# Ronnypetson/epivo

Hardware: NVIDIA B200
Metric: KITTI-shape frame-pairs/sec (match+E-RANSAC+pose+LM) (higher is better)
Workload: dtype u32-popc+f64

## Files before the change

epivo_b200/csrc/seq.cu:

```cuda
#include <stdlib.h>
#include <string.h>

#include <algorithm>
#include <vector>

#include "common.cuh"
#include "stages.cuh"

namespace {
constexpr int SEQ_CHUNK = 8192;
constexpr int SEQ_CHUNK_OVERLAP = 1024;
constexpr int SEQ_STAGES = 7;
constexpr int SEQ_MAX_CHUNKS = 256;
}

struct epivo_seq {
    epivo_ctx* ctx = nullptr;
    int max_frames = 0, kp = 0, stride = 0, chunk = SEQ_CHUNK;
    float* d_kps = nullptr;
    uint32_t* d_desc = nullptr;
    uint32_t* d_planes = nullptr;
    int32_t* d_counts = nullptr;
    bool counts_set = false;
    int32_t *d_fq = nullptr, *d_ft = nullptr;
    bool pairs_set = false;
    int max_pairs = 0, n_list = 0;
    int frames_hi = 0;
    int list_max = 0;
    std::vector<int32_t> h_fq, h_ft;
    int32_t *d_mq = nullptr, *d_mt = nullptr, *d_md = nullptr, *d_nmatch = nullptr;
    uint8_t *d_emask = nullptr, *d_pmask = nullptr;
    double *d_E = nullptr, *d_R = nullptr, *d_t = nullptr, *d_T = nullptr, *d_T0 = nullptr;
    int32_t *d_ninl = nullptr, *d_iters = nullptr, *d_nmodels = nullptr, *d_status = nullptr, *d_ngood = nullptr;
    int32_t *d_lmactive = nullptr, *d_lmiters = nullptr;
    epivo_lm_res* d_lmres = nullptr;
    epivo_pair_result* d_results = nullptr;
    uint32_t *d_rowkey = nullptr, *d_rowkey2 = nullptr, *d_colkey = nullptr;
    double *d_xn = nullptr, *d_xin = nullptr, *d_lmp = nullptr, *d_lmq = nullptr, *d_w = nullptr;
    float* d_err = nullptr;
    int32_t* d_reps = nullptr;
    char* d_esswork = nullptr;
    size_t esswork_bytes = 0;
    epivo_pair_result* h_results = nullptr;
    cudaEvent_t ev[SEQ_MAX_CHUNKS][SEQ_STAGES] = {};
    cudaEvent_t evk[SEQ_MAX_CHUNKS][2] = {};
    cudaEvent_t evp[SEQ_MAX_CHUNKS] = {};
    cudaEvent_t ev_begin = nullptr, ev_end = nullptr;
    cudaStream_t stream2 = nullptr;
    cudaStream_t stream3 = nullptr;
    cudaStream_t stream4 = nullptr;
    cudaEvent_t ev_piece[SEQ_MAX_CHUNKS] = {};
    int geo_mode = 0;
    cudaEvent_t ev_matched[SEQ_MAX_CHUNKS] = {};
    cudaEvent_t ev_geo_done = nullptr;
    int overlap = 0;
    int match_pad = 0;
    int last_mgroups = 0, last_ggroups = 0;
    int last_n_pairs = 0, last_first = 0;
    float* d_trk = nullptr;
    bool last_frames = false;
    std::vector<void*> allocs;
};

namespace {

template <typename T>
int seq_alloc(epivo_seq* s, T** p, size_t count) {
    epivo_ctx* ctx = s->ctx;
    void* q = nullptr;
    EPV_CUDA(ctx, cudaMalloc(&q, std::max<size_t>(count, 1) * sizeof(T)));
    s->allocs.push_back(q);
    *p = reinterpret_cast<T*>(q);
    return EPIVO_OK;
}

__global__ void lm_prep_kernel(int n_pairs, int stride, epivo_pipeline_params prm, const double* __restrict__ R,
                               const double* __restrict__ t, const int32_t* __restrict__ status,
                               const int32_t* __restrict__ n_inl, const int32_t* __restrict__ n_good,
                               const double* __restrict__ xin, double* __restrict__ T0, double* __restrict__ T,
                               double* __restrict__ lmp, double* __restrict__ lmq, double* __restrict__ w,
                               int32_t* __restrict__ active) {
    const int pair = blockIdx.x;
    if (pair >= n_pairs) return;
    const int tid = threadIdx.x;
    const int N = prm.lm_points;
    __shared__ double sT[16];
    if (tid == 0) {
        double Rm[9], tv[3];
        for (int i = 0; i < 9; ++i) Rm[i] = R[(int64_t)pair * 9 + i];
        for (int i = 0; i < 3; ++i) tv[i] = t[(int64_t)pair * 3 + i];
        const bool ok = status[pair] == 0;
        if (!ok || (Rm[0] + Rm[4] + Rm[8]) < prm.min_trace) {
            for (int i = 0; i < 9; ++i) Rm[i] = (i % 4 == 0) ? 1.0 : 0.0;
            for (int i = 0; i < 3; ++i) tv[i] = prm.fallback_t[i];
        }
        if (sqrt(tv[0] * tv[0] + tv[1] * tv[1] + tv[2] * tv[2]) < prm.min_t_norm)
            for (int i = 0; i < 3; ++i) tv[i] = prm.fallback_t[i];
        for (int i = 0; i < 3; ++i) {
            for (int j = 0; j < 3; ++j) sT[i * 4 + j] = Rm[i * 3 + j];
            sT[i * 4 + 3] = tv[i];
        }
        sT[12] = sT[13] = sT[14] = 0.0;
        sT[15] = 1.0;
        active[pair] = (ok && n_inl[pair] >= N && n_good[pair] >= N) ? 1 : 0;
        w[pair] = 1.0;
    }
    __syncthreads();
    if (tid < 16) {
        T0[(int64_t)pair * 16 + tid] = sT[tid];
        T[(int64_t)pair * 16 + tid] = sT[tid];
    }
    const double* x = xin + (int64_t)pair * 4 * stride;
    for (int i = tid; i < N; i += blockDim.x) {
        const bool have = i < n_inl[pair];
        double* p = lmp + ((int64_t)pair * N + i) * 3;
        double* q = lmq + ((int64_t)pair * N + i) * 3;
        p[0] = have ? x[i] : 1.0;
        p[1] = have ? x[stride + i] : 1.0;
        p[2] = 1.0;
        q[0] = have ? x[2 * stride + i] : 1.0;
        q[1] = have ? x[3 * stride + i] : 1.0;
        q[2] = 1.0;
    }
}

__device__ __forceinline__ double knorm(float u, double a, double b) { return __fma_rn((double)u, a, b); }

__global__ void __launch_bounds__(256) points_in_kernel(const float* __restrict__ p0, const float* __restrict__ p1,
                                                        const int32_t* __restrict__ counts, int max_pts, int stride,
                                                        double ax, double bx, double ay, double by,
                                                        double* __restrict__ xn, int32_t* __restrict__ nmatch,
                                                        int32_t* __restrict__ mq, int32_t* __restrict__ mt) {
    const int pair = blockIdx.y, i = blockIdx.x * 256 + threadIdx.x;
    const int n = min(max(counts[pair], 0), max_pts);
    if (i == 0) nmatch[pair] = n;
    if (i >= n) return;
    const float2 a = reinterpret_cast<const float2*>(p0)[(size_t)pair * max_pts + i];
    const float2 b = reinterpret_cast<const float2*>(p1)[(size_t)pair * max_pts + i];
    double* x = xn + (size_t)pair * 4 * stride;
    x[i] = knorm(a.x, ax, bx);
    x[stride + i] = knorm(a.y, ay, by);
    x[2 * stride + i] = knorm(b.x, ax, bx);
    x[3 * stride + i] = knorm(b.y, ay, by);
    mq[(size_t)pair * stride + i] = i;
    mt[(size_t)pair * stride + i] = i;
}

__global__ void __launch_bounds__(256) track_compact_kernel(const int32_t* __restrict__ meta, int n, const float* __restrict__ kps,
                                                            const int32_t* __restrict__ found, int kp,
                                                            const float* __restrict__ next, const uint8_t* __restrict__ status,
                                                            int stride, double ax, double bx, double ay, double by,
                                                            float* __restrict__ trk, double* __restrict__ xn,
                                                            int32_t* __restrict__ nmatch, int32_t* __restrict__ mq,
                                                            int32_t* __restrict__ mt, int32_t* __restrict__ md) {
    __shared__ int s_warp[8];
    __shared__ int s_carry;
    const int j = blockIdx.x, tid = threadIdx.x, lane = tid & 31, warp = tid >> 5;
    const int fq = meta[j], pair = meta[2 * n + j];
    const int cnt = min(found[fq], kp);
    const float2* c = reinterpret_cast<const float2*>(kps) + (size_t)fq * kp;
    const float2* nx = reinterpret_cast<const float2*>(next) + (size_t)j * kp;
    const uint8_t* st = status + (size_t)j * kp;
    float2* t0 = reinterpret_cast<float2*>(trk) + (size_t)pair * 2 * stride;
    float2* t1 = t0 + stride;
    double* x = xn + (size_t)pair * 4 * stride;
    const size_t mo = (size_t)pair * stride;
    if (tid == 0) s_carry = 0;
    __syncthreads();
    for (int base = 0; base < cnt; base += 256) {
        const int i = base + tid;
        const bool keep = i < cnt && st[i] == 1;
        const unsigned bal = __ballot_sync(0xFFFFFFFFu, keep);
        if (lane == 0) s_warp[warp] = __popc(bal);
        __syncthreads();
// ... 52 lines not shown
    r.lm_iters = ran ? lmiters[pair] : 0;
    r.lm_ran = ran ? 1 : 0;
    r.lm_reverted = revert ? 1 : 0;
    out[pair] = r;
}

}

extern "C" {

void epivo_pipeline_params_default(epivo_pipeline_params* p) {
    if (!p) return;
    memset(p, 0, sizeof(*p));
    p->norm = EPIVO_NORM_HAMMING2;
    p->match_mode = EPIVO_MATCH_CROSSCHECK;
    p->ratio = 0.8f;
    const double K[9] = {(double)718.8560f, 0.0, (double)607.1928f, 0.0, (double)718.8560f, (double)185.2157f,
                         0.0, 0.0, 1.0};
    memcpy(p->K, K, sizeof(K));
    p->method = EPIVO_RANSAC;
    p->prob = 0.99;
    p->threshold = 1.0;
    p->max_iters = 1000;
    p->dist_thresh = 50.0;
    p->min_trace = 3.0 * 0.9;
    p->fallback_t[0] = 0.1;
    p->fallback_t[1] = 0.1;
    p->fallback_t[2] = -0.9;
    p->min_t_norm = 1e-5;
    p->lm_points = 48;
    p->lm_lambda0 = 1e-2;
    p->lm_epsilon = 1e-8;
    p->lm_max_iters = 30;
    p->huber_delta = 1e-5;
    p->lm_revert = 1e-9;
}

int epivo_seq_create(epivo_ctx* ctx, epivo_seq** out, int max_frames, int kp_per_frame) {
    return epivo_seq_create_pairs(ctx, out, max_frames, kp_per_frame, max_frames - 1);
}

int epivo_seq_create_pairs(epivo_ctx* ctx, epivo_seq** out, int max_frames, int kp_per_frame, int max_pairs) {
    if (!ctx || !out) return EPIVO_ERR_INVALID;
    *out = nullptr;
    if (max_frames < 2 || kp_per_frame < 1) EPV_FAIL(ctx, EPIVO_ERR_INVALID, "need >= 2 frames and >= 1 keypoint");
    if (max_pairs < max_frames - 1) EPV_FAIL(ctx, EPIVO_ERR_INVALID, "max_pairs %d < max_frames - 1", max_pairs);
    if (kp_per_frame > (int)EPV_IDX_MASK) EPV_FAIL(ctx, EPIVO_ERR_UNSUPPORTED, "too many keypoints per frame");
    EPV_CUDA(ctx, cudaSetDevice(ctx->device));
    epivo_seq* s = new epivo_seq();
    s->ctx = ctx;
    s->max_frames = max_frames;
    s->kp = kp_per_frame;
    s->stride = (kp_per_frame + 31) / 32 * 32;
    s->max_pairs = max_pairs;
    s->n_list = max_frames - 1;
    const size_t F = max_frames, P = max_pairs, st = s->stride, kp = kp_per_frame;
    s->chunk = (int)std::min<size_t>(SEQ_CHUNK, P);
    const size_t C = P;
    int rc = 0;
#define A(ptr, count) if (!rc) rc = seq_alloc(s, &s->ptr, (count))
    A(d_kps, F * kp * 2);
    A(d_desc, F * kp * 8);
    A(d_planes, F * kp * 8);
    A(d_counts, F);
    A(d_fq, P); A(d_ft, P);
    A(d_mq, P * st); A(d_mt, P * st); A(d_md, P * st); A(d_nmatch, P);
    A(d_emask, P * st); A(d_pmask, P * st);
    A(d_E, P * 9); A(d_R, P * 9); A(d_t, P * 3); A(d_T, P * 16); A(d_T0, P * 16);
    A(d_ninl, P); A(d_iters, P); A(d_nmodels, P); A(d_status, P); A(d_ngood, P);
    A(d_lmactive, P); A(d_lmiters, P); A(d_lmres, P); A(d_results, P);
    A(d_rowkey, C * st); A(d_rowkey2, C * st); A(d_colkey, C * st);
    A(d_xn, C * 4 * st); A(d_xin, C * 4 * st);
    A(d_lmp, C * 64 * 3); A(d_lmq, C * 64 * 3); A(d_w, C);
    A(d_err, epv_essential_errbuf_floats((int)C, (int)st));
    A(d_reps, 2);
    s->esswork_bytes = epv_essential_work_bytes((int)std::min<size_t>(P, SEQ_CHUNK));
    A(d_esswork, s->esswork_bytes);
#undef A
    if (!rc && cudaMallocHost(&s->h_results, P * sizeof(epivo_pair_result)) != cudaSuccess) rc = EPIVO_ERR_CUDA;
    bool ev_ok = true;
    for (int c = 0; c < SEQ_MAX_CHUNKS && ev_ok; ++c)
    {
        for (int k = 0; k < SEQ_STAGES; ++k) ev_ok &= cudaEventCreate(&s->ev[c][k]) == cudaSuccess;
        for (int k = 0; k < 2; ++k) ev_ok &= cudaEventCreate(&s->evk[c][k]) == cudaSuccess;
        ev_ok &= cudaEventCreate(&s->evp[c]) == cudaSuccess;
    }
    for (int c = 0; c < SEQ_MAX_CHUNKS && ev_ok; ++c)
        ev_ok &= cudaEventCreateWithFlags(&s->ev_matched[c], cudaEventDisableTiming) == cudaSuccess;
    ev_ok = ev_ok && cudaEventCreate(&s->ev_begin) == cudaSuccess && cudaEventCreate(&s->ev_end) == cudaSuccess;
    ev_ok = ev_ok && cudaEventCreateWithFlags(&s->ev_geo_done, cudaEventDisableTiming) == cudaSuccess;
    {
        int lo = 0, hi = 0;
        cudaDeviceGetStreamPriorityRange(&lo, &hi);
        ev_ok = ev_ok && cudaStreamCreateWithPriority(&s->stream2, cudaStreamNonBlocking, hi) == cudaSuccess;
        ev_ok = ev_ok && cudaStreamCreateWithFlags(&s->stream3, cudaStreamNonBlocking) == cudaSuccess;
        ev_ok = ev_ok && cudaStreamCreateWithPriority(&s->stream4, cudaStreamNonBlocking, hi) == cudaSuccess;
        for (int c = 0; c < SEQ_MAX_CHUNKS && ev_ok; ++c)
            ev_ok &= cudaEventCreateWithFlags(&s->ev_piece[c], cudaEventDisableTiming) == cudaSuccess;
    }
    if (rc || !ev_ok) {
        epivo_seq_destroy(s);
        if (!rc) EPV_FAIL(ctx, EPIVO_ERR_CUDA, "event creation failed");
        return rc;
    }
    const int32_t reps[2] = {0, 0};
    EPV_CUDA(ctx, cudaMemcpyAsync(s->d_reps, reps, 8, cudaMemcpyHostToDevice, ctx->stream));
    {
        std::vector<int32_t> full((size_t)max_frames, kp_per_frame);
        EPV_CUDA(ctx, cudaMemcpyAsync(s->d_counts, full.data(), full.size() * 4, cudaMemcpyHostToDevice, ctx->stream));
        EPV_CUDA(ctx, cudaStreamSynchronize(ctx->stream));
    }
    rc = epivo_seq_set_pairs(s, 0, nullptr, nullptr);
    if (rc) { epivo_seq_destroy(s); return rc; }
    s->pairs_set = false;
    EPV_CUDA(ctx, cudaStreamSynchronize(ctx->stream));
    *out = s;
    return EPIVO_OK;
}

void epivo_seq_destroy(epivo_seq* s) {
    if (!s) return;
    cudaSetDevice(s->ctx->device);
    cudaStreamSynchronize(s->ctx->stream);
    for (void* p : s->allocs) cudaFree(p);
    if (s->h_results) cudaFreeHost(s->h_results);
    for (int c = 0; c < SEQ_MAX_CHUNKS; ++c)
        for (int k = 0; k < SEQ_STAGES; ++k)
            if (s->ev[c][k]) cudaEventDestroy(s->ev[c][k]);
    for (int c = 0; c < SEQ_MAX_CHUNKS; ++c)
        for (int k = 0; k < 2; ++k)
            if (s->evk[c][k]) cudaEventDestroy(s->evk[c][k]);
    for (int c = 0; c < SEQ_MAX_CHUNKS; ++c)
        if (s->evp[c]) cudaEventDestroy(s->evp[c]);
    for (int c = 0; c < SEQ_MAX_CHUNKS; ++c)
        if (s->ev_matched[c]) cudaEventDestroy(s->ev_matched[c]);
    if (s->ev_geo_done) cudaEventDestroy(s->ev_geo_done);
    if (s->stream2) { cudaStreamSynchronize(s->stream2); cudaStreamDestroy(s->stream2); }
    if (s->stream3) { cudaStreamSynchronize(s->stream3); cudaStreamDestroy(s->stream3); }
    if (s->stream4) { cudaStreamSynchronize(s->stream4); cudaStreamDestroy(s->stream4); }
    for (int c = 0; c < SEQ_MAX_CHUNKS; ++c)
        if (s->ev_piece[c]) cudaEventDestroy(s->ev_piece[c]);
    if (s->ev_begin) cudaEventDestroy(s->ev_begin);
    if (s->ev_end) cudaEventDestroy(s->ev_end);
    delete s;
}

int epivo_seq_upload(epivo_seq* s, int first_frame, int n_frames, const float* kps, const uint8_t* descs) {
    if (!s) return EPIVO_ERR_INVALID;
    epivo_ctx* ctx = s->ctx;
    if (first_frame < 0 || n_frames < 0 || first_frame + n_frames > s->max_frames || !kps || !descs)
        EPV_FAIL(ctx, EPIVO_ERR_INVALID, "frame range [%d,+%d) outside [0,%d)", first_frame, n_frames, s->max_frames);
    EPV_CUDA(ctx, cudaSetDevice(ctx->device));
    const size_t kp = s->kp;
    EPV_CUDA(ctx, cudaMemcpyAsync(s->d_kps + (size_t)first_frame * kp * 2, kps, (size_t)n_frames * kp * 8,
                                  cudaMemcpyHostToDevice, ctx->stream));
    EPV_CUDA(ctx, cudaMemcpyAsync(s->d_desc + (size_t)first_frame * kp * 8, descs, (size_t)n_frames * kp * 32,
                                  cudaMemcpyHostToDevice, ctx->stream));
    s->frames_hi = std::max(s->frames_hi, first_frame + n_frames);
    return EPIVO_OK;
}

int epivo_seq_set_pairs(epivo_seq* s, int n_pairs, const int32_t* fq, const int32_t* ft) {
    if (!s) return EPIVO_ERR_INVALID;
    epivo_ctx* ctx = s->ctx;
    std::vector<int32_t> h;
    if (n_pairs <= 0 || !fq || !ft) {
        n_pairs = s->max_frames - 1;
        h.resize((size_t)n_pairs * 2);
        for (int p = 0; p < n_pairs; ++p) { h[p] = p; h[(size_t)n_pairs + p] = p + 1; }
        s->pairs_set = false;
    } else {
        if (n_pairs > s->max_pairs) EPV_FAIL(ctx, EPIVO_ERR_INVALID, "%d pairs > capacity %d (epivo_seq_create_pairs)", n_pairs, s->max_pairs);
        h.resize((size_t)n_pairs * 2);
        int lmax = 0;
        for (int p = 0; p < n_pairs; ++p) {
            if (fq[p] < 0 || fq[p] >= s->max_frames || ft[p] < 0 || ft[p] >= s->max_frames)
                EPV_FAIL(ctx, EPIVO_ERR_INVALID, "pair %d = (%d,%d) outside [0,%d)", p, fq[p], ft[p], s->max_frames);
            h[p] = fq[p];
            h[(size_t)n_pairs + p] = ft[p];
            lmax = std::max(lmax, std::max(fq[p], ft[p]));
        }
        s->list_max = lmax;
        s->pairs_set = true;
    }
    s->h_fq.assign(h.begin(), h.begin() + n_pairs);
    s->h_ft.assign(h.begin() + n_pairs, h.end());
    EPV_CUDA(ctx, cudaSetDevice(ctx->device));
    EPV_CUDA(ctx, cudaMemcpyAsync(s->d_fq, h.data(), (size_t)n_pairs * 4, cudaMemcpyHostToDevice, ctx->stream));
    EPV_CUDA(ctx, cudaMemcpyAsync(s->d_ft, h.data() + n_pairs, (size_t)n_pairs * 4, cudaMemcpyHostToDevice, ctx->stream));
    EPV_CUDA(ctx, cudaStreamSynchronize(ctx->stream));
    s->n_list = n_pairs;
    return EPIVO_OK;
}

int epivo_seq_set_counts(epivo_seq* s, int first_frame, int n_frames, const int32_t* counts) {
    if (!s) return EPIVO_ERR_INVALID;
    epivo_ctx* ctx = s->ctx;
    if (first_frame < 0 || n_frames < 0 || first_frame + n_frames > s->max_frames || (n_frames > 0 && !counts))
        EPV_FAIL(ctx, EPIVO_ERR_INVALID, "frame range [%d,+%d) outside [0,%d)", first_frame, n_frames, s->max_frames);
    for (int i = 0; i < n_frames; ++i)
        if (counts[i] < 0 || counts[i] > s->kp) EPV_FAIL(ctx, EPIVO_ERR_INVALID, "counts[%d] = %d outside [0,%d]", i, counts[i], s->kp);
    EPV_CUDA(ctx, cudaSetDevice(ctx->device));
    EPV_CUDA(ctx, cudaMemcpyAsync(s->d_counts + first_frame, counts, (size_t)n_frames * 4, cudaMemcpyHostToDevice, ctx->stream));
    EPV_CUDA(ctx, cudaStreamSynchronize(ctx->stream));
    s->counts_set = true;
    return EPIVO_OK;
}

__global__ void __launch_bounds__(256) seq_orb_to_slots_kernel(const epivo_keypoint* __restrict__ kps, const uint32_t* __restrict__ desc,
                                                               const int32_t* __restrict__ found, int n_frames, int kp,
                                                               float* __restrict__ slot_kps, uint32_t* __restrict__ slot_desc,
                                                               int32_t* __restrict__ slot_counts) {
    const int f = blockIdx.y;
    const int n = min(found[f], kp);
    if (blockIdx.x == 0 && threadIdx.x == 0) slot_counts[f] = n;
    for (int i = blockIdx.x * 256 + threadIdx.x; i < n * 8; i += gridDim.x * 256) {
        const int k = i >> 3, w = i & 7;
        slot_desc[((size_t)f * kp + k) * 8 + w] = desc[((size_t)f * kp + k) * 8 + w];
        if (w < 2) slot_kps[((size_t)f * kp + k) * 2 + w] = w == 0 ? kps[(size_t)f * kp + k].x : kps[(size_t)f * kp + k].y;
    }
}

int epivo_seq_extract_orb(epivo_seq* s, int first_frame, int n_frames, const uint8_t* images, int rows, int cols,
                          int nfeatures, float scale_factor, int nlevels, int edge_threshold, int fast_threshold,
                          int32_t* counts_out) {
    if (!s) return EPIVO_ERR_INVALID;
    epivo_ctx* ctx = s->ctx;
    if (first_frame < 0 || n_frames < 0 || first_frame + n_frames > s->max_frames)
        EPV_FAIL(ctx, EPIVO_ERR_INVALID, "frame range [%d,+%d) outside [0,%d)", first_frame, n_frames, s->max_frames);
    if (n_frames == 0) return EPIVO_OK;
    if (!images || rows <= 0 || cols <= 0) EPV_FAIL(ctx, EPIVO_ERR_INVALID, "null or empty images");
    if (fast_threshold < 0 || fast_threshold > 255) EPV_FAIL(ctx, EPIVO_ERR_INVALID, "fast_threshold %d outside [0, 255]", fast_threshold);
    const int kp = s->kp;
    EpvOrbPlan plan;
    int rc = epv_orb_plan(ctx, n_frames, rows, cols, nfeatures, scale_factor, nlevels, edge_threshold, kp, &plan);
    if (rc) return rc;
    EPV_CUDA(ctx, cudaSetDevice(ctx->device));
    const size_t nk = (size_t)n_frames * kp;
    rc = epv_ws_reserve(ctx, epv_orb_work_bytes(plan) + nk * (sizeof(epivo_keypoint) + 32) + (size_t)n_frames * 4 + 4096);
    if (rc) return rc;
    rc = epv_pin_reserve(ctx, (plan.tab_entries + 1) * 4 + 512);
    if (rc) return rc;
    uint8_t* d_pyr = epv_ws_take<uint8_t>(ctx, plan.pyr_bytes);
    epivo_keypoint* d_kps = epv_ws_take<epivo_keypoint>(ctx, nk + 1);
    uint8_t* d_desc = epv_ws_take<uint8_t>(ctx, nk * 32 + 32);
    int32_t* d_found = epv_ws_take<int32_t>(ctx, n_frames);
    uint32_t* h_tab = epv_pin_take<uint32_t>(ctx, plan.tab_entries + 1);
    EPV_CUDA(ctx, cudaMemcpyAsync(d_pyr, images, (size_t)n_frames * rows * cols, cudaMemcpyHostToDevice, ctx->stream));
    rc = epv_orb_launch(ctx, plan, fast_threshold, d_pyr, d_kps, d_desc, d_found, h_tab);
    if (rc) return rc;
    seq_orb_to_slots_kernel<<<dim3(std::max(1, std::min((kp * 8 + 255) / 256, 64)), n_frames), 256, 0, ctx->stream>>>(
        d_kps, (const uint32_t*)d_desc, d_found, n_frames, kp, s->d_kps + (size_t)first_frame * kp * 2,
        s->d_desc + (size_t)first_frame * kp * 8, s->d_counts + first_frame);
    EPV_LAUNCHED(ctx);
    if (counts_out) EPV_CUDA(ctx, cudaMemcpyAsync(counts_out, d_found, (size_t)n_frames * 4, cudaMemcpyDeviceToHost, ctx->stream));
    EPV_CUDA(ctx, cudaStreamSynchronize(ctx->stream));
    s->counts_set = true;
    s->frames_hi = std::max(s->frames_hi, first_frame + n_frames);
    return EPIVO_OK;
}

int epivo_seq_set_overlap(epivo_seq* s, int overlap) {
    if (!s) return EPIVO_ERR_INVALID;
    s->overlap = overlap == 1 ? 1 : 0;
    s->geo_mode = overlap == 2 ? 2 : 0;
    return EPIVO_OK;
}

static int seq_run_geometry(epivo_seq* s, const epivo_pipeline_params* prm, int c, int p0, int np) {
    epivo_ctx* ctx = s->ctx;
    const int st = s->stride;
    const size_t o = (size_t)p0;
    int rc;
    EPV_CUDA(ctx, cudaEventRecord(s->ev[c][2], ctx->stream));
    EpvRange r_geo(ctx, "epivo: geometry (findEssentialMat + recoverPose + LM)");
    EssentialPlan ep{};
    ep.n_pairs = np;
    ep.stride = st;
    ep.xn = s->d_xn + o * 4 * st;
    ep.n = s->d_nmatch + p0;
    ep.method = prm->method;
    ep.prob = prm->prob;
    ep.thresh = prm->threshold / ((prm->K[0] + prm->K[4]) / 2.0);
    ep.max_iters = prm->max_iters;
    ep.samples = nullptr;
    ep.m = 0;
    ep.errbuf = s->d_err + epv_essential_errbuf_floats(p0, st);
    ep.E = s->d_E + o * 9;
    ep.mask = s->d_emask + o * st;
    ep.n_inliers = s->d_ninl + p0;
    ep.iters = s->d_iters + p0;
    ep.n_models = s->d_nmodels + p0;
    ep.status = s->d_status + p0;
    ep.xin = s->d_xin + o * 4 * st;
    ep.work = s->d_esswork;
    ep.work_bytes = s->esswork_bytes;
    ep.ev_presolved = s->evp[c];
    {
        EpvRange r(ctx, "epivo: findEssentialMat");
        rc = epv_essential_launch(ctx, ep);
    }
    if (rc) return rc;
    EPV_CUDA(ctx, cudaEventRecord(s->ev[c][3], ctx->stream));
    PosePlan pp{};
    pp.n_pairs = np;
    pp.stride = st;
    pp.E = s->d_E + o * 9;
    pp.xn = s->d_xin + o * 4 * st;
    pp.n = s->d_ninl + p0;
    pp.in_mask = nullptr;
    pp.dist_thresh = prm->dist_thresh;
    pp.R = s->d_R + o * 9;
    pp.t = s->d_t + o * 3;
    pp.mask = s->d_pmask + o * st;
    pp.n_good = s->d_ngood + p0;
    pp.skip = s->d_status + p0;
    {
        EpvRange r(ctx, "epivo: recoverPose");
        rc = epv_pose_launch(ctx, pp);
    }
    if (rc) return rc;
    EPV_CUDA(ctx, cudaEventRecord(s->ev[c][4], ctx->stream));
    lm_prep_kernel<<<np, 64, 0, ctx->stream>>>(np, st, *prm, s->d_R + o * 9, s->d_t + o * 3, s->d_status + p0,
                                               s->d_ninl + p0, s->d_ngood + p0, s->d_xin + o * 4 * st,
                                               s->d_T0 + o * 16, s->d_T + o * 16, s->d_lmp + o * 64 * 3,
                                               s->d_lmq + o * 64 * 3, s->d_w + p0, s->d_lmactive + p0);
    EPV_LAUNCHED(ctx);
    LmPlan lp{};
    lp.B = np;
    lp.n_zeta = 1;
    lp.n_rep = 1;
    lp.N = prm->lm_points;
    lp.reps = s->d_reps;
    lp.wreps = s->d_w + p0;
    lp.epsilon = prm->lm_epsilon;
    lp.lambda0 = prm->lm_lambda0;
    lp.huber_delta = prm->huber_delta;
    lp.max_iters = prm->lm_max_iters;
    lp.T0s = s->d_T + o * 16;
    lp.pr = s->d_lmp + o * 64 * 3;
    lp.p_r = s->d_lmq + o * 64 * 3;
    lp.out = s->d_lmres + p0;
    lp.iters = s->d_lmiters + p0;
    lp.active = s->d_lmactive + p0;
    lp.single_pair = 1;
    {
        EpvRange r(ctx, "epivo: Levenberg_Marquardt");
        rc = epv_lm_launch(ctx, lp);
    }
    if (rc) return rc;
    EPV_CUDA(ctx, cudaEventRecord(s->ev[c][5], ctx->stream));
    finish_kernel<<<(np + 127) / 128, 128, 0, ctx->stream>>>(
        np, *prm, s->d_E + o * 9, s->d_R + o * 9, s->d_t + o * 3, s->d_T0 + o * 16, s->d_T + o * 16, s->d_lmres + p0,
        s->d_lmiters + p0, s->d_lmactive + p0, s->d_nmatch + p0, s->d_ninl + p0, s->d_ngood + p0, s->d_iters + p0,
        s->d_nmodels + p0, s->d_results + p0);
    EPV_LAUNCHED(ctx);
    EPV_CUDA(ctx, cudaEventRecord(s->ev[c][6], ctx->stream));
    return EPIVO_OK;
}

static int seq_run_match(epivo_seq* s, const epivo_pipeline_params* prm, int c, int p0, int np, bool planes_ready = false) {
    epivo_ctx* ctx = s->ctx;
    const int kp = s->kp, st = s->stride;
    const size_t o = (size_t)p0;
    int rc;
    EPV_CUDA(ctx, cudaEventRecord(s->ev[c][0], ctx->stream));
    EpvRange r_match(ctx, "epivo: BFMatcher::match");
    MatchPlan mp{};
    mp.desc = s->d_desc + o * kp * 8;
    mp.planes = s->d_planes + o * kp * 8;
    mp.total_rows = (int64_t)(np + 1) * kp;
    mp.words = 8;
    mp.norm = prm->norm;
    mp.top2 = prm->match_mode == EPIVO_MATCH_RATIO;
    mp.n_pairs = np;
    mp.q0 = 0;
    mp.qs = kp;
    mp.t0 = kp;
    mp.ts = kp;
    mp.nq = kp;
    mp.nt = kp;
    mp.tsplits = 1;
    mp.rowkey = s->d_rowkey + o * st;
    mp.rowkey2 = s->d_rowkey2 + o * st;
    mp.colkey = s->d_colkey + o * st;
    mp.stride = st;
    mp.ev0 = s->evk[c][0];
    mp.ev1 = s->evk[c][1];
    mp.pad_smem = s->match_pad;
    const bool general = s->counts_set || s->pairs_set;
    bool prepass = true;
    if (general) {
        mp.desc = s->d_desc;
        mp.planes = s->d_planes;
        mp.fq = s->d_fq + p0;
        mp.ft = s->d_ft + p0;
        mp.counts = s->d_counts;
        if (s->pairs_set) {
            prepass = (c == 0);
            mp.prepass_row0 = 0;
            mp.total_rows = (int64_t)s->frames_hi * kp;
        } else {
            mp.prepass_row0 = (int64_t)p0 * kp;
        }
    }
    if (planes_ready) prepass = false;
    rc = epv_match_launch(ctx, mp, prepass);
    if (rc) return rc;
    EPV_CUDA(ctx, cudaEventRecord(s->ev[c][1], ctx->stream));
    FinalizePlan fp{};
    fp.n_pairs = np;
    fp.nq = kp;
    fp.nt = kp;
    fp.stride = st;
    fp.mode = prm->match_mode;
    fp.tsplits = 1;
    fp.ratio = prm->ratio;
    fp.rowkey = s->d_rowkey + o * st;
    fp.rowkey2 = s->d_rowkey2 + o * st;
    fp.colkey = s->d_colkey + o * st;
    fp.mq = s->d_mq + o * st;
    fp.mt = s->d_mt + o * st;
    fp.md = s->d_md + o * st;
    fp.md2 = nullptr;
    fp.n_matches = s->d_nmatch + p0;
    fp.kps = s->d_kps + o * kp * 2;
    fp.q0 = 0;
    fp.qs = kp;
    fp.t0 = kp;
    fp.ts = kp;
    fp.p0 = nullptr;
    fp.p1 = nullptr;
    fp.xn = s->d_xn + o * 4 * st;
    const double ax = 1.0 / prm->K[0], ay = 1.0 / prm->K[4];
    fp.ax = ax;
    fp.bx = -prm->K[2] * ax;
    fp.ay = ay;
    fp.by = -prm->K[5] * ay;
    if (general) {
        fp.kps = s->d_kps;
        fp.fq = s->d_fq + p0;
        fp.ft = s->d_ft + p0;
        fp.counts = s->d_counts;
    }
    rc = epv_finalize_launch(ctx, fp);
    if (rc) return rc;
    return EPIVO_OK;
}

__device__ __forceinline__ unsigned long long epv_globaltimer_ns() {
    unsigned long long t;
    asm volatile("mov.u64 %0, %%globaltimer;" : "=l"(t));
    return t;
}
__global__ void upload_delay_kernel(unsigned us) {
    const unsigned long long t0 = epv_globaltimer_ns();
    while (epv_globaltimer_ns() - t0 < (unsigned long long)us * 1000ull) __nanosleep(2000);
}

static int seq_execute(epivo_seq* s, const epivo_pipeline_params* prm, int first_pair, int n_pairs,
                       const float* h_kps, const uint8_t* h_desc, int n_frames_up) {
    epivo_ctx* ctx = s->ctx;
    if (first_pair < 0 || n_pairs < 0 || first_pair + n_pairs > s->n_list)
        EPV_FAIL(ctx, EPIVO_ERR_INVALID, "pair range [%d,+%d) outside [0,%d)", first_pair, n_pairs, s->n_list);
    if (prm->lm_points < 1 || prm->lm_points > 64) EPV_FAIL(ctx, EPIVO_ERR_UNSUPPORTED, "lm_points must be in [1,64]");
    if (prm->method != EPIVO_RANSAC && prm->method != EPIVO_LMEDS) EPV_FAIL(ctx, EPIVO_ERR_INVALID, "method");
    if (prm->match_mode < 0 || prm->match_mode > 2) EPV_FAIL(ctx, EPIVO_ERR_INVALID, "match_mode");
    if (prm->norm != EPIVO_NORM_HAMMING && prm->norm != EPIVO_NORM_HAMMING2) EPV_FAIL(ctx, EPIVO_ERR_INVALID, "norm");
    EPV_CUDA(ctx, cudaSetDevice(ctx->device));
    cudaStream_t main_stream = ctx->stream;
    EpvRange r_seq(ctx, h_kps ? "epivo_seq_process" : "epivo_seq_run");
    const bool upload_all = h_kps != nullptr && s->pairs_set;
    const bool upload = h_kps != nullptr && !upload_all;
    const bool overlap = s->overlap && !upload && !upload_all;
    if (upload || upload_all) s->frames_hi = std::max(s->frames_hi, first_pair + n_frames_up);
    if (s->pairs_set && s->frames_hi == 0) EPV_FAIL(ctx, EPIVO_ERR_INVALID, "pair list set but no frames uploaded");
    if (s->pairs_set && s->list_max >= s->frames_hi)
        EPV_FAIL(ctx, EPIVO_ERR_INVALID, "the pair list references frame %d but only frames [0,%d) have been uploaded",
                 s->list_max, s->frames_hi);
    constexpr int HALF = SEQ_MAX_CHUNKS / 2;
    std::vector<std::pair<int, int> > mg;
    {
        const int mchunk = overlap ? SEQ_CHUNK_OVERLAP : SEQ_CHUNK;
        int wave = upload ? epv_match_pairs_per_wave(ctx, s->kp) : mchunk;
        int max_pieces = HALF, cap_waves = 4;
        if (upload) {
            int div = 4;
            if (const char* e = getenv("EPIVO_UPLOAD_DIV")) div = std::max(1, atoi(e));
            wave = std::max(1, wave / div);
            if (const char* e = getenv("EPIVO_UPLOAD_PIECES")) max_pieces = std::min(HALF, std::max(1, atoi(e)));
            if (const char* e = getenv("EPIVO_UPLOAD_CAP")) cap_waves = std::max(1, atoi(e));
            while ((n_pairs + (int64_t)wave * cap_waves - 1) / ((int64_t)wave * cap_waves) + 2 > max_pieces && cap_waves < (1 << 20))
                cap_waves *= 2;
        }
        int p0 = first_pair, left = n_pairs, waves = 1;
        while (left > 0) {
            int np = upload ? wave * waves : mchunk;
            if (upload && ((int)mg.size() >= max_pieces - 1 || left - np < wave)) np = left;
            np = std::min(np, left);
            mg.push_back(std::make_pair(p0, np));
            p0 += np;
            left -= np;
            waves = std::min(2 * waves, cap_waves);
        }
    }
    const int gchunk = overlap ? SEQ_CHUNK_OVERLAP : SEQ_CHUNK;
    const int n_m = (int)mg.size(), n_g = (n_pairs + gchunk - 1) / gchunk;
    if (n_m > HALF || n_g > HALF) EPV_FAIL(ctx, EPIVO_ERR_UNSUPPORTED, "too many pair groups");
    s->last_mgroups = n_m;
    s->last_ggroups = n_g;
    s->last_frames = false;
    s->last_n_pairs = n_pairs;
    s->last_first = first_pair;
    int geo_mode = s->geo_mode;
    if (const char* e = getenv("EPIVO_GEO_MODE")) geo_mode = atoi(e);
    const bool interleave = upload && n_m >= 8 && geo_mode == 2;
    if (upload && getenv("EPIVO_DEBUG_SCHED"))
        fprintf(stderr, "[epivo dev %d] host-buffer call: %d pieces, interleave %d\n", ctx->device, n_m, (int)interleave);
    EPV_CUDA(ctx, cudaEventRecord(s->ev_begin, main_stream));
    int rc = EPIVO_OK;
    const size_t kp = s->kp;
    const bool planes_on_copy = upload && prm->norm == EPIVO_NORM_HAMMING2;
    if (upload) {
        EPV_CUDA(ctx, cudaStreamWaitEvent(s->stream2, s->ev_begin, 0));
        EPV_CUDA(ctx, cudaStreamWaitEvent(s->stream3, s->ev_begin, 0));
        const char* de = getenv("EPIVO_UPLOAD_DELAY_US");
        const int delay_us = de ? atoi(de) : 0;
        for (int c = 0; c < n_m; ++c) {
            const int p0 = mg[c].first, np = mg[c].second;
            const int f0 = (c == 0) ? p0 : p0 + 1;
            const int nf = p0 + np + 1 - f0;
            const size_t ho = (size_t)(f0 - first_pair);
            EPV_CUDA(ctx, cudaMemcpyAsync(s->d_kps + (size_t)f0 * kp * 2, h_kps + ho * kp * 2, (size_t)nf * kp * 8,
                                          cudaMemcpyHostToDevice, s->stream2));
            EPV_CUDA(ctx, cudaMemcpyAsync(s->d_desc + (size_t)f0 * kp * 8, h_desc + ho * kp * 32, (size_t)nf * kp * 32,
                                          cudaMemcpyHostToDevice, s->stream2));
            if (planes_on_copy) {
                rc = epv_planes_launch(ctx, s->d_desc + (size_t)f0 * kp * 8, s->d_planes + (size_t)f0 * kp * 8,
                                       (int64_t)nf * kp, 8, s->stream2);
                if (rc) return rc;
            }
            if (delay_us > 0) upload_delay_kernel<<<1, 1, 0, s->stream2>>>((unsigned)delay_us);
            EPV_CUDA(ctx, cudaEventRecord(s->ev_matched[c], s->stream2));
        }
        if (interleave) EPV_CUDA(ctx, cudaStreamWaitEvent(s->stream4, s->ev_begin, 0));
    }
    if (upload_all) {
        EPV_CUDA(ctx, cudaStreamWaitEvent(s->stream2, s->ev_begin, 0));
        EPV_CUDA(ctx, cudaMemcpyAsync(s->d_kps, h_kps, (size_t)n_frames_up * kp * 8, cudaMemcpyHostToDevice, s->stream2));
        EPV_CUDA(ctx, cudaMemcpyAsync(s->d_desc, h_desc, (size_t)n_frames_up * kp * 32, cudaMemcpyHostToDevice, s->stream2));
        EPV_CUDA(ctx, cudaEventRecord(s->ev_matched[0], s->stream2));
        EPV_CUDA(ctx, cudaStreamWaitEvent(main_stream, s->ev_matched[0], 0));
    }
    if (overlap) EPV_CUDA(ctx, cudaStreamWaitEvent(s->stream2, s->ev_begin, 0));
    int n_geo = 0;
    for (int c = 0; c < n_m && !rc; ++c) {
        const int p0 = mg[c].first, np = mg[c].second;
        cudaStream_t piece_stream = main_stream;
        if (upload) {
            piece_stream = (c & 1) ? s->stream3 : main_stream;
            EPV_CUDA(ctx, cudaStreamWaitEvent(piece_stream, s->ev_matched[c], 0));
        }
        ctx->stream = piece_stream;
        rc = seq_run_match(s, prm, c, p0, np, planes_on_copy);
        ctx->stream = main_stream;
        if (rc) break;
        if (interleave) {
            EPV_CUDA(ctx, cudaEventRecord(s->ev_piece[c], piece_stream));
            const int per = (n_m + 3) / 4;
            if ((c + 1) % per == 0 || c == n_m - 1) {
                const int c0 = (c / per) * per;
                const int gp0 = mg[c0].first, gnp = p0 + np - gp0;
                EPV_CUDA(ctx, cudaStreamWaitEvent(s->stream4, s->ev_piece[c], 0));
                if (c > 0) EPV_CUDA(ctx, cudaStreamWaitEvent(s->stream4, s->ev_piece[c - 1], 0));
                ctx->stream = s->stream4;
                rc = seq_run_geometry(s, prm, HALF + n_geo, gp0, gnp);
                ctx->stream = main_stream;
                if (rc) break;
                ++n_geo;
            }
        }
        if (overlap) {
            EPV_CUDA(ctx, cudaEventRecord(s->ev_matched[c], main_stream));
            EPV_CUDA(ctx, cudaStreamWaitEvent(s->stream2, s->ev_matched[c], 0));
            ctx->stream = s->stream2;
            rc = seq_run_geometry(s, prm, HALF + c, p0, np);
            ctx->stream = main_stream;
        }
    }
    if (upload && n_m > 1 && !rc) {
        EPV_CUDA(ctx, cudaEventRecord(s->ev_geo_done, s->stream3));
        EPV_CUDA(ctx, cudaStreamWaitEvent(main_stream, s->ev_geo_done, 0));
    }
    ctx->stream = main_stream;
    if (rc) return rc;
    if (interleave) {
        s->last_ggroups = n_geo;
        EPV_CUDA(ctx, cudaEventRecord(s->ev_geo_done, s->stream4));
        EPV_CUDA(ctx, cudaStreamWaitEvent(main_stream, s->ev_geo_done, 0));
    } else if (overlap) {
        EPV_CUDA(ctx, cudaEventRecord(s->ev_geo_done, s->stream2));
        EPV_CUDA(ctx, cudaStreamWaitEvent(main_stream, s->ev_geo_done, 0));
    } else {
        for (int c = 0; c < n_g && !rc; ++c) {
            const int p0 = first_pair + c * gchunk;
            const int np = std::min(gchunk, first_pair + n_pairs - p0);
            rc = seq_run_geometry(s, prm, HALF + c, p0, np);
        }
        if (rc) return rc;
    }
    EPV_CUDA(ctx, cudaEventRecord(s->ev_end, main_stream));
    return EPIVO_OK;
}

int epivo_seq_run(epivo_seq* s, const epivo_pipeline_params* prm, int first_pair, int n_pairs) {
    if (!s || !prm) return EPIVO_ERR_INVALID;
    return seq_execute(s, prm, first_pair, n_pairs, nullptr, nullptr, 0);
}

int epivo_seq_process(epivo_seq* s, const epivo_pipeline_params* prm, int n_frames, const float* kps,
                      const uint8_t* descs, epivo_pair_result* out) {
    if (!s || !prm) return EPIVO_ERR_INVALID;
    epivo_ctx* ctx = s->ctx;
    if (!kps || !descs || !out) EPV_FAIL(ctx, EPIVO_ERR_INVALID, "null buffer");
    if (n_frames < 2 || n_frames > s->max_frames) EPV_FAIL(ctx, EPIVO_ERR_INVALID, "n_frames %d outside [2,%d]", n_frames, s->max_frames);
    if (s->pairs_set && s->list_max >= n_frames)
        EPV_FAIL(ctx, EPIVO_ERR_INVALID, "the pair list references frame %d but only %d frames are given", s->list_max, n_frames);
    const int n_pairs = s->pairs_set ? s->n_list : n_frames - 1;
    int rc = seq_execute(s, prm, 0, n_pairs, kps, descs, n_frames);
    if (rc) return rc;
    return epivo_seq_download(s, out, 0, n_pairs);
}

int epivo_seq_process_points(epivo_seq* s, const epivo_pipeline_params* prm, int n_pairs, const float* p0, const float* p1,
                             const int32_t* counts, int max_pts, epivo_pair_result* out) {
    if (!s || !prm) return EPIVO_ERR_INVALID;
    epivo_ctx* ctx = s->ctx;
    if (n_pairs < 0 || n_pairs > s->n_list) EPV_FAIL(ctx, EPIVO_ERR_INVALID, "n_pairs %d outside [0,%d]", n_pairs, s->n_list);
    if (n_pairs == 0) return EPIVO_OK;
    if (!p0 || !p1 || !counts || !out) EPV_FAIL(ctx, EPIVO_ERR_INVALID, "null buffer");
    if (max_pts < 1 || max_pts > s->kp) EPV_FAIL(ctx, EPIVO_ERR_INVALID, "max_pts %d outside [1,%d]", max_pts, s->kp);
    if (prm->lm_points < 1 || prm->lm_points > 64) EPV_FAIL(ctx, EPIVO_ERR_UNSUPPORTED, "lm_points must be in [1,64]");
    if (prm->method != EPIVO_RANSAC && prm->method != EPIVO_LMEDS) EPV_FAIL(ctx, EPIVO_ERR_INVALID, "method");
    for (int i = 0; i < n_pairs; ++i)
        if (counts[i] < 0 || counts[i] > max_pts) EPV_FAIL(ctx, EPIVO_ERR_INVALID, "counts[%d] = %d outside [0,%d]", i, counts[i], max_pts);
    EPV_CUDA(ctx, cudaSetDevice(ctx->device));
    EpvRange r_seq(ctx, "epivo_seq_process_points");
    const size_t np = (size_t)n_pairs * max_pts;
    int rc = epv_ws_reserve(ctx, np * 16 + (size_t)n_pairs * 4 + 4096);
    if (rc) return rc;
    float* d_p0 = epv_ws_take<float>(ctx, np * 2);
    float* d_p1 = epv_ws_take<float>(ctx, np * 2);
    int32_t* d_cnt = epv_ws_take<int32_t>(ctx, n_pairs);
    cudaStream_t st = ctx->stream;
    EPV_CUDA(ctx, cudaEventRecord(s->ev_begin, st));
    EPV_CUDA(ctx, cudaMemcpyAsync(d_p0, p0, np * 8, cudaMemcpyHostToDevice, st));
    EPV_CUDA(ctx, cudaMemcpyAsync(d_p1, p1, np * 8, cudaMemcpyHostToDevice, st));
    EPV_CUDA(ctx, cudaMemcpyAsync(d_cnt, counts, (size_t)n_pairs * 4, cudaMemcpyHostToDevice, st));
    const double ax = 1.0 / prm->K[0], ay = 1.0 / prm->K[4];
    points_in_kernel<<<dim3((max_pts + 255) / 256, n_pairs), 256, 0, st>>>(d_p0, d_p1, d_cnt, max_pts, s->stride, ax,
                                                                            -prm->K[2] * ax, ay, -prm->K[5] * ay, s->d_xn,
                                                                            s->d_nmatch, s->d_mq, s->d_mt);
    EPV_LAUNCHED(ctx);
    constexpr int HALF = SEQ_MAX_CHUNKS / 2;
    const int n_g = (n_pairs + SEQ_CHUNK - 1) / SEQ_CHUNK;
    if (n_g > HALF) EPV_FAIL(ctx, EPIVO_ERR_UNSUPPORTED, "too many pair groups");
    s->last_mgroups = 0;
    s->last_ggroups = n_g;
    s->last_n_pairs = n_pairs;
    s->last_first = 0;
    s->last_frames = false;
    for (int c = 0; c < n_g; ++c) {
        const int g0 = c * SEQ_CHUNK, gn = std::min(SEQ_CHUNK, n_pairs - g0);
        rc = seq_run_geometry(s, prm, HALF + c, g0, gn);
        if (rc) return rc;
    }
    EPV_CUDA(ctx, cudaEventRecord(s->ev_end, st));
    return epivo_seq_download(s, out, 0, n_pairs);
}

namespace {
constexpr int FRAMES_MAX_WINDOW = 256;
constexpr size_t FRAMES_WS_BUDGET = (size_t)3 << 29;
constexpr int LK_WINDOW = 21, LK_MAX_LEVEL = 3, LK_MAX_COUNT = 30;
constexpr double LK_EPSILON = 0.01, LK_MIN_EIG = 1e-4;

struct FramesWs {
    size_t src, img, maps, fast, lk, kps;
    size_t total() const { return src + img + maps + fast + lk + kps; }
};
FramesWs frames_ws(int g, int rows, int cols, int R, int C, bool maps, int kp) {
    FramesWs w;
    w.src = maps ? epv_align((size_t)g * rows * cols) : 0;
    w.img = epv_align((size_t)g * R * C);
    w.maps = maps ? epv_align((size_t)R * C * 4) + epv_align((size_t)R * C * 2) : 0;
    w.fast = epv_align(epv_fast_work_bytes(g, R, C));
    w.lk = epv_align(epv_lk_work_bytes(g, R, C, LK_MAX_LEVEL));
    w.kps = epv_align((size_t)g * kp * 8);
    return w;
}
}

int epivo_seq_process_frames(epivo_seq* s, const epivo_pipeline_params* prm, int n_frames, const uint8_t* images, int rows,
                             int cols, const int16_t* map_xy, const uint16_t* map_frac, int drows, int dcols,
                             int fast_threshold, int32_t* corners_out, epivo_pair_result* out) {
    if (!s || !prm) return EPIVO_ERR_INVALID;
    epivo_ctx* ctx = s->ctx;
    if (!images || !out) EPV_FAIL(ctx, EPIVO_ERR_INVALID, "null buffer");
    if (n_frames < 2 || n_frames > s->max_frames) EPV_FAIL(ctx, EPIVO_ERR_INVALID, "n_frames %d outside [2,%d]", n_frames, s->max_frames);
    if (rows <= 0 || cols <= 0) EPV_FAIL(ctx, EPIVO_ERR_INVALID, "empty frames (%d x %d)", cols, rows);
    const bool maps = map_xy != nullptr || map_frac != nullptr;
    if (maps && (!map_xy || !map_frac || drows <= 0 || dcols <= 0))
        EPV_FAIL(ctx, EPIVO_ERR_INVALID, "remap needs both maps and a positive size (%d x %d)", dcols, drows);
    const int R = maps ? drows : rows, C = maps ? dcols : cols;
    if (R <= LK_WINDOW || C <= LK_WINDOW)
        EPV_FAIL(ctx, EPIVO_ERR_UNSUPPORTED, "image %d x %d not larger than the %d x %d LK window", C, R, LK_WINDOW, LK_WINDOW);
    if (fast_threshold < 0 || fast_threshold > 255) EPV_FAIL(ctx, EPIVO_ERR_INVALID, "fast_threshold %d outside [0, 255]", fast_threshold);
// ... 261 lines not shown
```

Measured before the change: 274,300.

## Compute descriptor bit-planes once at upload and drop per-match prepass

Builds the bit-plane transposed descriptors whenever descriptors are uploaded or extracted, and tracks their validity with a planes_ok flag. The matcher then never runs its planes prepass, which removes repeated planes recomputation from each match call, especially on the device-resident path where the prepass ran on every call or piece. In exchange, planes are now computed even for norms that may not use them, and correctness depends on the validity flag being kept in sync.

```diff
diff --git a/epivo_b200/csrc/seq.cu b/epivo_b200/csrc/seq.cu
--- a/epivo_b200/csrc/seq.cu
+++ b/epivo_b200/csrc/seq.cu
@@ -20,6 +20,7 @@
     float* d_kps = nullptr;
     uint32_t* d_desc = nullptr;
     uint32_t* d_planes = nullptr;
+    bool planes_ok = false;
     int32_t* d_counts = nullptr;
     bool counts_set = false;
     int32_t *d_fq = nullptr, *d_ft = nullptr;
@@ -378,10 +379,16 @@
         EPV_FAIL(ctx, EPIVO_ERR_INVALID, "frame range [%d,+%d) outside [0,%d)", first_frame, n_frames, s->max_frames);
     EPV_CUDA(ctx, cudaSetDevice(ctx->device));
     const size_t kp = s->kp;
+    const bool planes_ok = s->planes_ok;
+    s->planes_ok = false;
     EPV_CUDA(ctx, cudaMemcpyAsync(s->d_kps + (size_t)first_frame * kp * 2, kps, (size_t)n_frames * kp * 8,
                                   cudaMemcpyHostToDevice, ctx->stream));
     EPV_CUDA(ctx, cudaMemcpyAsync(s->d_desc + (size_t)first_frame * kp * 8, descs, (size_t)n_frames * kp * 32,
                                   cudaMemcpyHostToDevice, ctx->stream));
+    int rc = epv_planes_launch(ctx, s->d_desc + (size_t)first_frame * kp * 8, s->d_planes + (size_t)first_frame * kp * 8,
+                               (int64_t)n_frames * kp, 8, ctx->stream);
+    if (rc) return rc;
+    s->planes_ok = planes_ok;
     s->frames_hi = std::max(s->frames_hi, first_frame + n_frames);
     return EPIVO_OK;
 }
@@ -462,6 +469,8 @@
     int rc = epv_orb_plan(ctx, n_frames, rows, cols, nfeatures, scale_factor, nlevels, edge_threshold, kp, &plan);
     if (rc) return rc;
     EPV_CUDA(ctx, cudaSetDevice(ctx->device));
+    const bool planes_ok = s->planes_ok;
+    s->planes_ok = false;
     const size_t nk = (size_t)n_frames * kp;
     rc = epv_ws_reserve(ctx, epv_orb_work_bytes(plan) + nk * (sizeof(epivo_keypoint) + 32) + (size_t)n_frames * 4 + 4096);
     if (rc) return rc;
@@ -479,8 +488,12 @@
         d_kps, (const uint32_t*)d_desc, d_found, n_frames, kp, s->d_kps + (size_t)first_frame * kp * 2,
         s->d_desc + (size_t)first_frame * kp * 8, s->d_counts + first_frame);
     EPV_LAUNCHED(ctx);
+    rc = epv_planes_launch(ctx, s->d_desc + (size_t)first_frame * kp * 8, s->d_planes + (size_t)first_frame * kp * 8,
+                           (int64_t)n_frames * kp, 8, ctx->stream);
+    if (rc) return rc;
     if (counts_out) EPV_CUDA(ctx, cudaMemcpyAsync(counts_out, d_found, (size_t)n_frames * 4, cudaMemcpyDeviceToHost, ctx->stream));
     EPV_CUDA(ctx, cudaStreamSynchronize(ctx->stream));
+    s->planes_ok = planes_ok;
     s->counts_set = true;
     s->frames_hi = std::max(s->frames_hi, first_frame + n_frames);
     return EPIVO_OK;
@@ -585,7 +598,7 @@
     return EPIVO_OK;
 }
 
-static int seq_run_match(epivo_seq* s, const epivo_pipeline_params* prm, int c, int p0, int np, bool planes_ready = false) {
+static int seq_run_match(epivo_seq* s, const epivo_pipeline_params* prm, int c, int p0, int np) {
     epivo_ctx* ctx = s->ctx;
     const int kp = s->kp, st = s->stride;
     const size_t o = (size_t)p0;
@@ -595,7 +608,6 @@
     MatchPlan mp{};
     mp.desc = s->d_desc + o * kp * 8;
     mp.planes = s->d_planes + o * kp * 8;
-    mp.total_rows = (int64_t)(np + 1) * kp;
     mp.words = 8;
     mp.norm = prm->norm;
     mp.top2 = prm->match_mode == EPIVO_MATCH_RATIO;
@@ -615,23 +627,14 @@
     mp.ev1 = s->evk[c][1];
     mp.pad_smem = s->match_pad;
     const bool general = s->counts_set || s->pairs_set;
-    bool prepass = true;
     if (general) {
         mp.desc = s->d_desc;
         mp.planes = s->d_planes;
         mp.fq = s->d_fq + p0;
         mp.ft = s->d_ft + p0;
         mp.counts = s->d_counts;
-        if (s->pairs_set) {
-            prepass = (c == 0);
-            mp.prepass_row0 = 0;
-            mp.total_rows = (int64_t)s->frames_hi * kp;
-        } else {
-            mp.prepass_row0 = (int64_t)p0 * kp;
-        }
-    }
-    if (planes_ready) prepass = false;
-    rc = epv_match_launch(ctx, mp, prepass);
+    }
+    rc = epv_match_launch(ctx, mp, false);
     if (rc) return rc;
     EPV_CUDA(ctx, cudaEventRecord(s->ev[c][1], ctx->stream));
     FinalizePlan fp{};
@@ -743,10 +746,15 @@
     const bool interleave = upload && n_m >= 8 && geo_mode == 2;
     if (upload && getenv("EPIVO_DEBUG_SCHED"))
         fprintf(stderr, "[epivo dev %d] host-buffer call: %d pieces, interleave %d\n", ctx->device, n_m, (int)interleave);
-    EPV_CUDA(ctx, cudaEventRecord(s->ev_begin, main_stream));
     int rc = EPIVO_OK;
     const size_t kp = s->kp;
-    const bool planes_on_copy = upload && prm->norm == EPIVO_NORM_HAMMING2;
+    if (!s->planes_ok) {
+        rc = epv_planes_launch(ctx, s->d_desc, s->d_planes, (int64_t)s->max_frames * s->kp, 8, main_stream);
+        if (rc) return rc;
+        s->planes_ok = true;
+    }
+    EPV_CUDA(ctx, cudaEventRecord(s->ev_begin, main_stream));
+    if (upload || upload_all) s->planes_ok = false;
     if (upload) {
         EPV_CUDA(ctx, cudaStreamWaitEvent(s->stream2, s->ev_begin, 0));
         EPV_CUDA(ctx, cudaStreamWaitEvent(s->stream3, s->ev_begin, 0));
@@ -761,11 +769,9 @@
                                           cudaMemcpyHostToDevice, s->stream2));
             EPV_CUDA(ctx, cudaMemcpyAsync(s->d_desc + (size_t)f0 * kp * 8, h_desc + ho * kp * 32, (size_t)nf * kp * 32,
                                           cudaMemcpyHostToDevice, s->stream2));
-            if (planes_on_copy) {
-                rc = epv_planes_launch(ctx, s->d_desc + (size_t)f0 * kp * 8, s->d_planes + (size_t)f0 * kp * 8,
-                                       (int64_t)nf * kp, 8, s->stream2);
-                if (rc) return rc;
-            }
+            rc = epv_planes_launch(ctx, s->d_desc + (size_t)f0 * kp * 8, s->d_planes + (size_t)f0 * kp * 8,
+                                   (int64_t)nf * kp, 8, s->stream2);
+            if (rc) return rc;
             if (delay_us > 0) upload_delay_kernel<<<1, 1, 0, s->stream2>>>((unsigned)delay_us);
             EPV_CUDA(ctx, cudaEventRecord(s->ev_matched[c], s->stream2));
         }
@@ -775,9 +781,12 @@
         EPV_CUDA(ctx, cudaStreamWaitEvent(s->stream2, s->ev_begin, 0));
         EPV_CUDA(ctx, cudaMemcpyAsync(s->d_kps, h_kps, (size_t)n_frames_up * kp * 8, cudaMemcpyHostToDevice, s->stream2));
         EPV_CUDA(ctx, cudaMemcpyAsync(s->d_desc, h_desc, (size_t)n_frames_up * kp * 32, cudaMemcpyHostToDevice, s->stream2));
+        rc = epv_planes_launch(ctx, s->d_desc, s->d_planes, (int64_t)n_frames_up * kp, 8, s->stream2);
+        if (rc) return rc;
         EPV_CUDA(ctx, cudaEventRecord(s->ev_matched[0], s->stream2));
         EPV_CUDA(ctx, cudaStreamWaitEvent(main_stream, s->ev_matched[0], 0));
     }
+    s->planes_ok = true;
     if (overlap) EPV_CUDA(ctx, cudaStreamWaitEvent(s->stream2, s->ev_begin, 0));
     int n_geo = 0;
     for (int c = 0; c < n_m && !rc; ++c) {
@@ -788,7 +797,7 @@
             EPV_CUDA(ctx, cudaStreamWaitEvent(piece_stream, s->ev_matched[c], 0));
         }
         ctx->stream = piece_stream;
-        rc = seq_run_match(s, prm, c, p0, np, planes_on_copy);
+        rc = seq_run_match(s, prm, c, p0, np);
         ctx->stream = main_stream;
         if (rc) break;
         if (interleave) {
```

New measurement: 276,600 (median of 6 runs). Within noise of the previous version (+0.8%).
